# wenhao728/VORTA

Hardware: AMD Instinct MI355X
Metric: video_tokens_per_sec (routed-attention denoising step, HunyuanVideo 720p 129f) (higher is better)
Workload: dtype fp16

## Files before the change

### vorta_amd/csrc/attn_fwd.hip

```cpp
#include <hip/hip_runtime.h>
#include <stdint.h>

#include "vorta_hip.h"
#include "common.h"

#include "attn_common.h"
#include "attn_fwd_diag.inc"

namespace {
using namespace vorta_attn;

template <typename T, int NW>
__global__ __launch_bounds__(NW * 64, 2) void attn_fwd_kernel(const Params p) {
  using V8 = typename MF<T>::v8;
  using V4 = typename MF<T>::v4;
  constexpr int NT = NW * 64;
  constexpr int QB = NW * 32;
  constexpr int CH = (KVB * 16) / NT;
  constexpr int ROWSTEP = NT / 16;

  __shared__ __attribute__((aligned(16))) char smem[2 * BUF_BYTES];

  const int wg = live_order(p, blockIdx.x, gridDim.x, p.xcd_remap);
  const int sp = wg % p.n_splits;
  const int rest = wg / p.n_splits;
  const int n_qb = p.n_groups * p.blocks_per_group;
  const int qb = rest % n_qb;
  const int y = rest / n_qb;
  if (p.n_heads_dev && y >= *p.n_heads_dev) return;
  const int head = p.head_list ? p.head_list[y] : y;
  int grp, p0, pend;
  q_block_of(p, qb, QB, grp, p0, pend);

  const int tid = threadIdx.x;
  const int lane = tid & 63;
  const int wave = __builtin_amdgcn_readfirstlane(tid >> 6);
  const int r32 = lane & 31;
  const int hh = lane >> 5;

  const int n_kv = p.n_kv_dev ? max(1, min(*p.n_kv_dev, p.n_kv)) : p.n_kv;
  const int q_valid = p.q_valid_dev ? min(*p.q_valid_dev, p.q_valid) : p.q_valid;
  const int nblk_total = (n_kv + KVB - 1) / KVB;
  const int blk0 = sp * p.blocks_per_split;
  const int blk1 = min(blk0 + p.blocks_per_split, nblk_total);

  const int wrow0 = p0 + wave * 32;
  const bool wave_active = wrow0 < pend;
  const int my_p = wrow0 + r32;
  const bool row_ok = my_p < pend;
  const int ld_p = min(my_p, pend - 1);
  const int32_t* q_rows = p.q_rows ? p.q_rows + (int64_t)y * p.q_rows_sh : nullptr;
  const int64_t my_row = q_rows ? (int64_t)q_rows[ld_p] : (int64_t)(p.q_row_offset + ld_p);

  V8 qf[8];
  {
    const char* qp = p.q + (int64_t)head * p.q_sh + my_row * p.q_ss + hh * 16;
#pragma unroll
    for (int ks = 0; ks < 8; ++ks) qf[ks] = *(const V8*)(qp + ks * 32);
  }

  const int32_t* kv_rows =
      p.kv_rows ? p.kv_rows + (int64_t)y * p.kv_rows_sh + (int64_t)grp * p.kv_rows_sg : nullptr;
  const char* kbase = p.k + (int64_t)head * p.k_sh + (tid & 15) * 16;
  const char* vbase = p.v + (int64_t)head * p.v_sh + (tid & 15) * 16;
  const int lrow0 = tid >> 4;
  const int lcc = tid & 15;
  int k_wr[CH], v_wr[CH];
#pragma unroll
  for (int i = 0; i < CH; ++i) {
    const int row = lrow0 + i * ROWSTEP;
    k_wr[i] = row * ROWB + ((lcc ^ (row & 15)) << 4);
    v_wr[i] = TILE_BYTES + row * ROWB + ((lcc ^ ((row & 3) << 2)) << 4);
  }
  u32x4 kreg[CH], vreg[CH];
  int64_t nrow[CH];
#define FETCH_ROWS(blk_)                                                          \
  _Pragma("unroll") for (int i_ = 0; i_ < CH; ++i_) {                             \
    const int pos_ = min((blk_) * KVB + lrow0 + i_ * ROWSTEP, n_kv - 1);          \
    nrow[i_] = kv_rows ? (int64_t)kv_rows[pos_] : (int64_t)(p.kv_row_offset + pos_); \
  }
#define ISSUE_LOADS()                                                             \
  _Pragma("unroll") for (int i_ = 0; i_ < CH; ++i_) {                             \
    kreg[i_] = *(const u32x4*)(kbase + nrow[i_] * p.k_ss);                        \
    vreg[i_] = *(const u32x4*)(vbase + nrow[i_] * p.v_ss);                        \
  }
#define WRITE_LDS(buf_)                                                           \
  _Pragma("unroll") for (int i_ = 0; i_ < CH; ++i_) {                             \
    *(u32x4*)(smem + (buf_) * BUF_BYTES + k_wr[i_]) = kreg[i_];                   \
    *(u32x4*)(smem + (buf_) * BUF_BYTES + v_wr[i_]) = vreg[i_];                   \
  }

  int k_rd[8];
#pragma unroll
  for (int ks = 0; ks < 8; ++ks) k_rd[ks] = r32 * ROWB + (((2 * ks + hh) ^ (r32 & 15)) << 4);
  int v_rd[4];
  {
    const int g = lane >> 4, i16 = lane & 15, q4 = i16 >> 2, pp = i16 & 3;
#pragma unroll
    for (int dt = 0; dt < 4; ++dt)
      v_rd[dt] = TILE_BYTES + (4 * (g >> 1) + q4) * ROWB + ((dt ^ q4) << 6) + 32 * (g & 1) + 8 * pp;
  }

  f32x16 o[4];
#pragma unroll
  for (int dt = 0; dt < 4; ++dt)
#pragma unroll
    for (int i = 0; i < 16; ++i) o[dt][i] = 0.f;
  float m_run = -1e30f, l_run = 0.f;
  const float c = p.scale_log2;

  if (blk0 < blk1) {
    FETCH_ROWS(blk0);
    ISSUE_LOADS();
    if (blk0 + 1 < blk1) { FETCH_ROWS(blk0 + 1); }
    WRITE_LDS(0);
    if (blk0 + 1 < blk1) { ISSUE_LOADS(); }
    if (blk0 + 2 < blk1) { FETCH_ROWS(blk0 + 2); }
    __syncthreads();
  }

  for (int blk = blk0; blk < blk1; ++blk) {
    const int buf = (blk - blk0) & 1;
    const char* sb = smem + buf * BUF_BYTES;
    V8 pb[4];
    if (wave_active) {
      f32x16 s0, s1;
#pragma unroll
      for (int i = 0; i < 16; ++i) { s0[i] = 0.f; s1[i] = 0.f; }
#pragma unroll
      for (int ks = 0; ks < 8; ++ks) {
        const V8 k0 = *(const V8*)(sb + k_rd[ks]);
        const V8 k1 = *(const V8*)(sb + k_rd[ks] + 32 * ROWB);
        s0 = MF<T>::mfma(k0, qf[ks], s0);
        s1 = MF<T>::mfma(k1, qf[ks], s1);
      }
      const int kv0 = blk * KVB;
      if (kv0 + KVB > n_kv) {
#pragma unroll
        for (int i = 0; i < 16; ++i) {
          const int row = (i & 3) + 8 * (i >> 2) + 4 * hh;
          if (kv0 + row >= n_kv) s0[i] = -INFINITY;
          if (kv0 + 32 + row >= n_kv) s1[i] = -INFINITY;
        }
      }
      float mx = s0[0];
#pragma unroll
      for (int i = 1; i < 16; ++i) mx = fmaxf(mx, s0[i]);
#pragma unroll
      for (int i = 0; i < 16; ++i) mx = fmaxf(mx, s1[i]);
      mx = half_max(mx);
      const float m_new = fmaxf(m_run, mx);
      if (!__all(m_new == m_run)) {
        const float alpha = __builtin_amdgcn_exp2f((m_run - m_new) * c);
#pragma unroll
        for (int dt = 0; dt < 4; ++dt)
#pragma unroll
          for (int i = 0; i < 16; ++i) o[dt][i] *= alpha;
        l_run *= alpha;
        m_run = m_new;
      }
      const float mc = m_run * c;
      float lsum = 0.f;
#pragma unroll
      for (int i = 0; i < 16; ++i) {
        s0[i] = __builtin_amdgcn_exp2f(fmaf(s0[i], c, -mc));
        s1[i] = __builtin_amdgcn_exp2f(fmaf(s1[i], c, -mc));
        lsum += s0[i] + s1[i];
      }
      l_run += lsum;
#pragma unroll
      for (int j = 0; j < 8; ++j) {
        pb[0][j] = (T)s0[j];
        pb[1][j] = (T)s0[8 + j];
        pb[2][j] = (T)s1[j];
        pb[3][j] = (T)s1[8 + j];
      }
    }
    if (blk + 1 < blk1) {
      WRITE_LDS(buf ^ 1);
      if (blk + 2 < blk1) { ISSUE_LOADS(); }
      if (blk + 3 < blk1) { FETCH_ROWS(blk + 3); }
    }
    if (wave_active) {
#pragma unroll
      for (int dt = 0; dt < 4; ++dt) {
#pragma unroll
        for (int kg = 0; kg < 4; ++kg) {
          const V4 lo = MF<T>::tr(sb + v_rd[dt] + (16 * kg) * ROWB);
          const V4 hi = MF<T>::tr(sb + v_rd[dt] + (16 * kg + 8) * ROWB);
          V8 vf;
#pragma unroll
          for (int j = 0; j < 4; ++j) { vf[j] = lo[j]; vf[4 + j] = hi[j]; }
          o[dt] = MF<T>::mfma(vf, pb[kg], o[dt]);
        }
      }
    }
    __syncthreads();
  }

  if (!wave_active) return;
  const float l_tot = half_sum(l_run);
  if (p.n_splits > 1) {
    if (row_ok) {
      const int64_t slot = ((int64_t)y * p.n_splits + sp) * p.n_q + my_p;
      float* wo = p.ws_o + slot * D;
#pragma unroll
      for (int dt = 0; dt < 4; ++dt)
#pragma unroll
        for (int rg = 0; rg < 4; ++rg) {
          f32x4 v = {o[dt][4 * rg], o[dt][4 * rg + 1], o[dt][4 * rg + 2], o[dt][4 * rg + 3]};
          *(f32x4*)(wo + 32 * dt + 8 * rg + 4 * hh) = v;
        }
      if (hh == 0) {
        p.ws_ml[slot * 2] = m_run * c;
        p.ws_ml[slot * 2 + 1] = l_tot;
      }
    }
    return;
  }
  if (!row_ok) return;
  const float inv = (my_p < q_valid && l_tot > 0.f) ? 1.f / l_tot : 0.f;
  uint2 packed[16];
#pragma unroll
  for (int dt = 0; dt < 4; ++dt)
#pragma unroll
    for (int rg = 0; rg < 4; ++rg) {
      V4 t;
#pragma unroll
      for (int j = 0; j < 4; ++j) t[j] = (T)(o[dt][4 * rg + j] * inv);
      packed[dt * 4 + rg] = *(uint2*)&t;
    }
  char* obase = p.o + (int64_t)head * p.o_sh + hh * 8;
  auto store_row = [&](int64_t row) {
    char* op = obase + row * p.o_ss;
#pragma unroll
    for (int dt = 0; dt < 4; ++dt)
#pragma unroll
      for (int rg = 0; rg < 4; ++rg) *(uint2*)(op + (32 * dt + 8 * rg) * 2) = packed[dt * 4 + rg];
  };
  store_row(my_row);
  if (p.dup_rows && my_p < p.n_dup_pos) {
    const int32_t* dr = p.dup_rows + (int64_t)y * p.dup_rows_sh + (int64_t)my_p * p.n_dup;
    for (int i = 0; i < p.n_dup; ++i) store_row((int64_t)dr[i]);
  }
}

constexpr int RING = 2;

template <typename T, int NW, bool KVTAB, int NS>
__device__ __forceinline__ void attn_pipe_dma_body(const Params& p, char* __restrict__ smem, const int wg) {
  static_assert(NS == 2, "ring depth");
  TRACE_ENTRY_()
  using V8 = typename MF<T>::v8;
  using V4 = typename MF<T>::v4;
  constexpr int NT = NW * 64;
  constexpr int QB = NW * 32;
  constexpr int CH = (KVB * 16) / NT;
  constexpr int ROWSTEP = NT / 16;
#ifndef VORTA_KPRE
#define VORTA_KPRE 2
#endif
  constexpr int KPRE = (NW == 4 && KVTAB && VORTA_KPRE > 1) ? 1 : VORTA_KPRE;
  const int sp = wg % p.n_splits;
  const int rest = wg / p.n_splits;
  const int n_qb = p.n_groups * p.blocks_per_group;
  const int qb = rest % n_qb;
  const int y = rest / n_qb;
  if (p.n_heads_dev && y >= *p.n_heads_dev) return;
  const int head = p.head_list ? p.head_list[y] : y;
  int grp, p0, pend;
  q_block_of(p, qb, QB, grp, p0, pend);

  const int tid = threadIdx.x;
  const int lane = tid & 63;
  const int wave = __builtin_amdgcn_readfirstlane(tid >> 6);
  const int r32 = lane & 31;
  const int hh = lane >> 5;

  const int n_kv = p.n_kv_dev ? max(1, min(*p.n_kv_dev, p.n_kv)) : p.n_kv;
  const int q_valid = p.q_valid_dev ? min(*p.q_valid_dev, p.q_valid) : p.q_valid;
  const int nblk_total = (n_kv + KVB - 1) / KVB;
  const int blk0 = sp * p.blocks_per_split;
  const int blk1 = min(blk0 + p.blocks_per_split, nblk_total);

  const int wrow0 = p0 + wave * 32;
  const bool wave_active = wrow0 < pend;
  const int my_p = wrow0 + r32;
  const bool row_ok = my_p < pend;
  const int ld_p = min(my_p, pend - 1);
  const int32_t* q_rows = p.q_rows ? p.q_rows + (int64_t)y * p.q_rows_sh : nullptr;
  const int64_t my_row = q_rows ? (int64_t)q_rows[ld_p] : (int64_t)(p.q_row_offset + ld_p);

  V8 qf[8];
  {
    const char* qp = p.q + (int64_t)head * p.q_sh + my_row * p.q_ss + hh * 16;
#pragma unroll
    for (int ks = 0; ks < 8; ++ks) {
      const V8 raw = *(const V8*)(qp + ks * 32);
#pragma unroll
      for (int i = 0; i < 8; ++i) qf[ks][i] = (T)((float)raw[i] * p.scale_log2);
    }
  }

  const int32_t* kv_rows =
      p.kv_rows ? p.kv_rows + (int64_t)y * p.kv_rows_sh + (int64_t)grp * p.kv_rows_sg : nullptr;
  const char* kbase = p.k + (int64_t)head * p.k_sh + (tid & 15) * 16;
  const char* vbase = p.v + (int64_t)head * p.v_sh + (tid & 15) * 16;
  const int lrow0 = tid >> 4;
  const int lcc = tid & 15;
  const __amdgpu_buffer_rsrc_t k_rsrc = __builtin_amdgcn_make_buffer_rsrc(
      (void*)(p.k + (int64_t)head * p.k_sh), 0, 0x7fffffff, 0x00020000);
  const __amdgpu_buffer_rsrc_t v_rsrc = __builtin_amdgcn_make_buffer_rsrc(
      (void*)(p.v + (int64_t)head * p.v_sh), 0, 0x7fffffff, 0x00020000);
  const int k_ss32 = (int)p.k_ss, v_ss32 = (int)p.v_ss;
  int k_col[CH], v_col[CH];
#pragma unroll
  for (int i = 0; i < CH; ++i) {
    const int row = 4 * (CH * wave + i) + (lane >> 4);
    k_col[i] = ((lane & 15) ^ (row & 15)) << 4;
    v_col[i] = ((lane & 15) ^ ((row & 3) << 2)) << 4;
  }
  int rowK[CH], rowV[CH];
  int posK[CH];
#define ROWS_OF(dst_, blk_)                                                       \
  _Pragma("unroll") for (int i_ = 0; i_ < CH; ++i_) {                             \
    const int pos_ = min((blk_) * KVB + 4 * (CH * wave + i_) + (lane >> 4), n_kv - 1); \
    if constexpr (KVTAB) dst_[i_] = kv_rows[pos_];                                \
    else dst_[i_] = p.kv_row_offset + pos_;                                       \
  }
#define DMA_K(par_) _Pragma("unroll") for (int i_ = 0; i_ < CH; ++i_) __builtin_amdgcn_raw_ptr_buffer_load_lds(   \
      k_rsrc, (LDS_AS void*)(smem + (par_) * TILE_BYTES + (CH * wave + i_) * 1024), 16,                            \
      (int)__umul24((unsigned)rowK[i_], (unsigned)k_ss32) + k_col[i_], 0, 0, 0);
#define DMA_V(par_) _Pragma("unroll") for (int i_ = 0; i_ < CH; ++i_) __builtin_amdgcn_raw_ptr_buffer_load_lds(   \
      v_rsrc, (LDS_AS void*)(smem + (NS + (par_)) * TILE_BYTES + (CH * wave + i_) * 1024), 16,                     \
      (int)__umul24((unsigned)rowV[i_], (unsigned)v_ss32) + v_col[i_], 0, 0, 0);

  int k_rd[8];
#pragma unroll
  for (int ks = 0; ks < 8; ++ks) k_rd[ks] = r32 * ROWB + (((2 * ks + hh) ^ (r32 & 15)) << 4);
  int v_rd[4];
  {
    const int g = lane >> 4, i16 = lane & 15, q4 = i16 >> 2, pp = i16 & 3;
#pragma unroll
    for (int dt = 0; dt < 4; ++dt)
      v_rd[dt] = NS * TILE_BYTES + (4 * (g >> 1) + q4) * ROWB + ((dt ^ q4) << 6) + 32 * (g & 1) + 8 * pp;
  }

  f32x16 o[4];
#pragma unroll
  for (int dt = 0; dt < 4; ++dt)
#pragma unroll
    for (int i = 0; i < 16; ++i) o[dt][i] = 0.f;
  float m_run = -1e30f, l_run = 0.f;
  const float defer = p.defer_log2;
  f32x16 sA0, sA1, sB0, sB1;
  f32x16 minit;
#pragma unroll
  for (int i = 0; i < 16; ++i) minit[i] = 0.f;
  float mx_cur = -1e30f;

#define QK(d0_, d1_, par_)                                                        \
  {                                                                               \
    _Pragma("unroll") for (int ks_ = 0; ks_ < 8; ++ks_) {                         \
      const V8 k0_ = *(const V8*)(smem + (par_) * TILE_BYTES + k_rd[ks_]);        \
      const V8 k1_ = *(const V8*)(smem + (par_) * TILE_BYTES + k_rd[ks_] + 32 * ROWB); \
      d0_ = MF<T>::mfma(k0_, qf[ks_], ks_ == 0 ? minit : d0_);                    \
      d1_ = MF<T>::mfma(k1_, qf[ks_], ks_ == 0 ? minit : d1_);                    \
    }                                                                             \
  }
#define ROW_MAX(dst_, a_, b_)                                                      \
  {                                                                               \
    float mx_ = a_[0];                                                            \
    _Pragma("unroll") for (int i_ = 1; i_ < 16; ++i_) mx_ = fmaxf(mx_, a_[i_]);   \
    _Pragma("unroll") for (int i_ = 0; i_ < 16; ++i_) mx_ = fmaxf(mx_, b_[i_]);   \
    dst_ = half_max(mx_);                                                         \
  }
#define ROW_MAX_POS(dst_, a_, b_)                                                  \
  {                                                                               \
    int m0_ = max(max(__float_as_int(a_[0]), __float_as_int(a_[1])), __float_as_int(a_[2])); \
    int m1_ = max(max(__float_as_int(b_[0]), __float_as_int(b_[1])), __float_as_int(b_[2])); \
    _Pragma("unroll") for (int i_ = 3; i_ < 15; i_ += 2) {                        \
      m0_ = max(max(m0_, __float_as_int(a_[i_])), __float_as_int(a_[i_ + 1]));    \
      m1_ = max(max(m1_, __float_as_int(b_[i_])), __float_as_int(b_[i_ + 1]));    \
    }                                                                             \
    m0_ = max(max(m0_, __float_as_int(a_[15])), __float_as_int(b_[15]));          \
    m0_ = max(m0_, m1_);                                                          \
    auto r_ = __builtin_amdgcn_permlane32_swap((unsigned)m0_, (unsigned)m0_, false, false); \
    dst_ = __int_as_float(max((int)r_[0], (int)r_[1]));                           \
  }
#define QK_PRE(d0_, d1_, par_)                                                    \
  {                                                                               \
    _Pragma("unroll") for (int ks_ = 0; ks_ < 8; ++ks_) {                         \
      V8 k0_, k1_;                                                                \
      if (ks_ < KPRE) { k0_ = kpre_[ks_][0]; k1_ = kpre_[ks_][1]; }               \
      else {                                                                      \
        k0_ = *(const V8*)(smem + (par_) * TILE_BYTES + k_rd[ks_]);               \
        k1_ = *(const V8*)(smem + (par_) * TILE_BYTES + k_rd[ks_] + 32 * ROWB);   \
      }                                                                           \
      d0_ = MF<T>::mfma(k0_, qf[ks_], ks_ == 0 ? minit : d0_);                    \
      d1_ = MF<T>::mfma(k1_, qf[ks_], ks_ == 0 ? minit : d1_);                    \
    }                                                                             \
  }
#define RAISE_REF(g_, c0_, c1_)                                                   \
  {                                                                               \
    const float alpha_ = __builtin_amdgcn_exp2f(-(g_));                           \
    _Pragma("unroll") for (int dt_ = 0; dt_ < 4; ++dt_)                           \
      _Pragma("unroll") for (int i_ = 0; i_ < 16; ++i_) o[dt_][i_] *= alpha_;     \
    l_run *= alpha_;                                                              \
    m_run += (g_);                                                                \
    _Pragma("unroll") for (int i_ = 0; i_ < 16; ++i_) { c0_[i_] -= (g_); c1_[i_] -= (g_); minit[i_] = -m_run; } \
    asm volatile("" : "+v"(minit));                                               \
  }
#define STAGE_DMA(kfree_, vfree_, j_)                                             \
  DMA_K(kfree_)                                                                   \
  DMA_V(vfree_)                                                                   \
  _Pragma("unroll") for (int i_ = 0; i_ < CH; ++i_) rowV[i_] = rowK[i_];          \
  if constexpr (NW == 8) {                                                        \
    _Pragma("unroll") for (int i_ = 0; i_ < CH; ++i_) {                           \
      posK[i_] += KVB;                                                            \
      const int pos_ = min(posK[i_], n_kv - 1);                                   \
      if constexpr (KVTAB) rowK[i_] = kv_rows[pos_];                              \
      else rowK[i_] = p.kv_row_offset + pos_;                                     \
    }                                                                             \
  } else {  \
    ROWS_OF(rowK, (j_) + NS + 1)                                                  \
  }                                                                               \
  __builtin_amdgcn_sched_barrier(0);
  TRACE_VARS_()
#ifndef STEP_SYNC
#define STEP_SYNC() asm volatile("s_waitcnt vmcnt(0) lgkmcnt(0)\n\ts_barrier" ::: "memory");
#endif

#ifndef VORTA_SCHED
#define VORTA_SCHED 1
#endif
#if VORTA_SCHED == 1
#define SCHED_RECIPE()                                                            \
  _Pragma("unroll") for (int g_ = 0; g_ < 16; ++g_) {                             \
    __builtin_amdgcn_sched_group_barrier(0x008, 1, 0);                            \
    __builtin_amdgcn_sched_group_barrier(0x100, 1, 0);                            \
    __builtin_amdgcn_sched_group_barrier(0x400, 2, 0);                            \
    __builtin_amdgcn_sched_group_barrier(0x002, 2, 0);                            \
  }                                                                               \
  _Pragma("unroll") for (int g_ = 0; g_ < 16; ++g_) {                             \
    __builtin_amdgcn_sched_group_barrier(0x008, 1, 0);                            \
    __builtin_amdgcn_sched_group_barrier(0x100, 2, 0);                            \
    __builtin_amdgcn_sched_group_barrier(0x002, 4, 0);                            \
  }
#else
#define SCHED_RECIPE()
#endif
#define STEP(c0_, c1_, n0_, n1_, kcur_, knext_, vfree_, j_)                       \
  {  \
    STAGE_DMA(kcur_, vfree_, j_)                                                  \
    STEP_BODY(c0_, c1_, n0_, n1_, kcur_, knext_, j_)                              \
    STEP_SYNC()                                                                   \
  }
#define STEP_BODY(c0_, c1_, n0_, n1_, kcur_, knext_, j_)                          \
  {                                                                               \
    if (wave_active) {                                                            \
      V8 kpre_[KPRE > 0 ? KPRE : 1][2];                                                          \
      _Pragma("unroll") for (int ks_ = 0; ks_ < KPRE; ++ks_) {                    \
        kpre_[ks_][0] = *(const V8*)(smem + (knext_) * TILE_BYTES + k_rd[ks_]);   \
        kpre_[ks_][1] = *(const V8*)(smem + (knext_) * TILE_BYTES + k_rd[ks_] + 32 * ROWB); \
      }                                                                           \
       \
       \
      if ((j_) * KVB + KVB > n_kv) {                                              \
        int h4_ = 4 * hh;  \
        asm volatile("" : "+v"(h4_));                                             \
        _Pragma("unroll") for (int i_ = 0; i_ < 16; ++i_) {                       \
          const int row_ = (i_ & 3) + 8 * (i_ >> 2) + h4_;                        \
          if ((j_) * KVB + row_ >= n_kv) c0_[i_] = -INFINITY;                     \
          if ((j_) * KVB + 32 + row_ >= n_kv) c1_[i_] = -INFINITY;                \
        }                                                                         \
        ROW_MAX(mx_cur, c0_, c1_)                                                 \
      }                                                                           \
       \
       \
       \
      if (!__all(mx_cur <= defer)) {                                              \
        const float g_ = fmaxf(mx_cur, 0.f);                                      \
        RAISE_REF(g_, c0_, c1_)                                                   \
      }                                                                           \
      V8 pb_[4];                                                                  \
      QK_PRE(n0_, n1_, knext_)     \
      float lsum_ = 0.f;                                                          \
      _Pragma("unroll") for (int i_ = 0; i_ < 16; ++i_) {                         \
        c0_[i_] = __builtin_amdgcn_exp2f(c0_[i_]);                                \
        c1_[i_] = __builtin_amdgcn_exp2f(c1_[i_]);                                \
        lsum_ += c0_[i_] + c1_[i_];                                               \
      }                                                                           \
      l_run += lsum_;                                                             \
      _Pragma("unroll") for (int e_ = 0; e_ < 8; ++e_) {                          \
        pb_[0][e_] = (T)c0_[e_];                                                  \
        pb_[1][e_] = (T)c0_[8 + e_];                                              \
        pb_[2][e_] = (T)c1_[e_];                                                  \
        pb_[3][e_] = (T)c1_[8 + e_];                                              \
      }                                                                           \
      _Pragma("unroll") for (int dt_ = 0; dt_ < 4; ++dt_) {                       \
        _Pragma("unroll") for (int kg_ = 0; kg_ < 4; ++kg_) {                     \
          const V4 lo_ = MF<T>::tr(smem + (kcur_) * TILE_BYTES + v_rd[dt_] + (16 * kg_) * ROWB); \
          const V4 hi_ = MF<T>::tr(smem + (kcur_) * TILE_BYTES + v_rd[dt_] + (16 * kg_ + 8) * ROWB); \
          V8 vf_;                                                                 \
          _Pragma("unroll") for (int e_ = 0; e_ < 4; ++e_) { vf_[e_] = lo_[e_]; vf_[4 + e_] = hi_[e_]; } \
          o[dt_] = MF<T>::mfma(vf_, pb_[kg_], o[dt_]);                            \
        }                                                                         \
      }                                                                           \
      ROW_MAX_POS(mx_cur, n0_, n1_)  \
      SCHED_RECIPE()                                                              \
    }                                                                             \
  }

  if (blk0 < blk1) {
    ROWS_OF(rowK, blk0)
    _Pragma("unroll") for (int i_ = 0; i_ < CH; ++i_) rowV[i_] = rowK[i_];
    DMA_K(0)
    DMA_V(0)
    ROWS_OF(rowK, blk0 + 1)
    DMA_K(1)
    _Pragma("unroll") for (int i_ = 0; i_ < CH; ++i_) rowV[i_] = rowK[i_];
    ROWS_OF(rowK, blk0 + NS)
    _Pragma("unroll") for (int i_ = 0; i_ < CH; ++i_) posK[i_] = (blk0 + NS) * KVB + 4 * (CH * wave + i_) + (lane >> 4);
    __syncthreads();
    if (wave_active) {
      QK(sA0, sA1, 0)
      if (blk0 * KVB + KVB > n_kv) {
#pragma unroll
        for (int i = 0; i < 16; ++i) {
          const int row = (i & 3) + 8 * (i >> 2) + 4 * hh;
          if (blk0 * KVB + row >= n_kv) sA0[i] = -INFINITY;
          if (blk0 * KVB + 32 + row >= n_kv) sA1[i] = -INFINITY;
        }
      }
      ROW_MAX(mx_cur, sA0, sA1)
      m_run = mx_cur;
#pragma unroll
      for (int i = 0; i < 16; ++i) { sA0[i] -= m_run; sA1[i] -= m_run; minit[i] = -m_run; }
      asm volatile("" : "+v"(minit));
      mx_cur = 0.f;
    }
    __syncthreads();
  }
  for (int blk = blk0; blk < blk1; blk += 2) {
    STEP(sA0, sA1, sB0, sB1, 0, 1, 1, blk)
    if (blk + 1 >= blk1) break;
    STEP(sB0, sB1, sA0, sA1, 1, 0, 0, blk + 1)
  }
#undef QK
#undef QK_PRE
#undef ROW_MAX
#undef ROW_MAX_POS
#undef RAISE_REF
#undef STEP
#undef STEP_BODY
#undef STAGE_DMA
#undef STEP_SYNC
#undef ROWS_OF
#undef DMA_K
#undef DMA_V

  TRACE_FLUSH_()
  if (!wave_active) return;
  const float l_tot = half_sum(l_run);
  if (p.n_splits > 1) {
    if (row_ok) {
      const int64_t slot = ((int64_t)y * p.n_splits + sp) * p.n_q + my_p;
      float* wo = p.ws_o + slot * D;
#pragma unroll
      for (int dt = 0; dt < 4; ++dt)
#pragma unroll
        for (int rg = 0; rg < 4; ++rg) {
          f32x4 v = {o[dt][4 * rg], o[dt][4 * rg + 1], o[dt][4 * rg + 2], o[dt][4 * rg + 3]};
          *(f32x4*)(wo + 32 * dt + 8 * rg + 4 * hh) = v;
        }
      if (hh == 0) {
        p.ws_ml[slot * 2] = m_run;
        p.ws_ml[slot * 2 + 1] = l_tot;
      }
    }
    return;
  }
  if (!row_ok) return;
  const float inv = (my_p < q_valid && l_tot > 0.f) ? 1.f / l_tot : 0.f;
  uint2 packed[16];
#pragma unroll
  for (int dt = 0; dt < 4; ++dt)
#pragma unroll
    for (int rg = 0; rg < 4; ++rg) {
      V4 t;
#pragma unroll
      for (int j = 0; j < 4; ++j) t[j] = (T)(o[dt][4 * rg + j] * inv);
      packed[dt * 4 + rg] = *(uint2*)&t;
    }
  char* obase = p.o + (int64_t)head * p.o_sh + hh * 8;
  auto store_row = [&](int64_t row) {
    char* op = obase + row * p.o_ss;
#pragma unroll
    for (int dt = 0; dt < 4; ++dt)
#pragma unroll
      for (int rg = 0; rg < 4; ++rg) *(uint2*)(op + (32 * dt + 8 * rg) * 2) = packed[dt * 4 + rg];
  };
  store_row(my_row);
  if (p.dup_rows && my_p < p.n_dup_pos) {
    const int32_t* dr = p.dup_rows + (int64_t)y * p.dup_rows_sh + (int64_t)my_p * p.n_dup;
    for (int i = 0; i < p.n_dup; ++i) store_row((int64_t)dr[i]);
  }
}


template <typename T, int NW, bool KVTAB>
__global__ __launch_bounds__(NW * 64, 2) void attn_fwd_pipe_kernel(const Params p) {
#if defined(__HIP_DEVICE_COMPILE__)
  constexpr int NS = RING;
  __shared__ __attribute__((aligned(16))) char smem[2 * NS * TILE_BYTES];
  const int wg = live_order(p, blockIdx.x, gridDim.x, p.xcd_remap);
  attn_pipe_dma_body<T, NW, KVTAB, NS>(p, smem, wg);
#endif
}


template <typename T>
__global__ __launch_bounds__(512, 2) void attn_fwd_multi_kernel(const MultiOf<Params> mp) {
#if defined(__HIP_DEVICE_COMPILE__)
  __shared__ __attribute__((aligned(16))) char smem[2 * RING * TILE_BYTES];
  int wg;
  const Params& p = segment_of(mp, blockIdx.x, wg);
  if (p.kv_rows) attn_pipe_dma_body<T, 8, true, RING>(p, smem, wg);
  else attn_pipe_dma_body<T, 8, false, RING>(p, smem, wg);
#endif
}

}

int vorta_attn::fill_params(const vorta_attn_args* a, Params& p, int& block_rows, int in_esize, int v_esize, int k_esize) {
  if (v_esize == 0) v_esize = in_esize;
  if (k_esize == 0) k_esize = in_esize;
  if (!a || a->struct_size != sizeof(vorta_attn_args)) return VORTA_EINVAL;
  if (in_esize == 2 ? (a->dtype != VORTA_BF16 && a->dtype != VORTA_FP16) : a->dtype != VORTA_FP8E4M3) return VORTA_EUNSUPPORTED;
  if (a->head_dim != D) return VORTA_EUNSUPPORTED;
  if (a->n_heads < 0 || a->n_q < 0 || a->n_kv < 0) return VORTA_EINVAL;
  if (a->n_heads == 0 || a->n_q == 0) { block_rows = 0; p.n_groups = 0; p.blocks_per_group = 0; p.n_heads = 0; return VORTA_OK; }
  if (a->n_kv == 0) return VORTA_EINVAL;
  if (!a->q.ptr || !a->k.ptr || !a->v.ptr || !a->o.ptr) return VORTA_EINVAL;
  const vorta_tensor* ts[4] = {&a->q, &a->k, &a->v, &a->o};
  for (int i = 0; i < 4; ++i) {
    const vorta_tensor* t = ts[i];
    const int al = 16 / (i == 0 ? in_esize : i == 1 ? k_esize : i == 2 ? v_esize : 2);
    if (((uintptr_t)t->ptr & 15) || (t->stride_s % al) || (t->stride_h % al) || t->stride_s < D) return VORTA_EINVAL;
  }
  if (a->n_splits < 1 || a->n_splits > 1024) return VORTA_EINVAL;
  if (!(a->scale > 0.f)) return VORTA_EINVAL;
  if (a->n_splits > 1 && (!a->ws_o || !a->ws_ml)) return VORTA_EINVAL;
  if (a->q_group_len < 0 || a->q_valid < 0) return VORTA_EINVAL;
  if (a->dup_rows && (a->n_dup < 0 || a->n_dup_pos < 0 || a->n_dup_pos > a->n_q)) return VORTA_EINVAL;
  if (a->block_rows != 0 && a->block_rows != 128 && a->block_rows != 256) return VORTA_EINVAL;
  if (a->variant < 0 || a->variant > 2) return VORTA_EINVAL;
  if (a->variant != 1 && (a->k.stride_s * k_esize >= (1 << 24) || a->v.stride_s * v_esize >= (1 << 24))) return VORTA_EUNSUPPORTED;
  if (a->variant != 1 && !a->kv_rows) {
    const int64_t last = (int64_t)a->kv_row_offset + a->n_kv;
    const int64_t ks = a->k.stride_s * k_esize, vs = a->v.stride_s * v_esize;
    const int64_t ss = ks > vs ? ks : vs;
    if (last >= (1 << 24) || last * ss > 0x7fffffffll) return VORTA_EUNSUPPORTED;
  }
  p.q = (const char*)a->q.ptr; p.k = (const char*)a->k.ptr; p.v = (const char*)a->v.ptr; p.o = (char*)a->o.ptr;
  p.q_sh = a->q.stride_h * in_esize; p.k_sh = a->k.stride_h * k_esize; p.v_sh = a->v.stride_h * v_esize; p.o_sh = a->o.stride_h * 2;
  p.q_ss = a->q.stride_s * in_esize; p.k_ss = a->k.stride_s * k_esize; p.v_ss = a->v.stride_s * v_esize; p.o_ss = a->o.stride_s * 2;
  p.head_list = a->head_list; p.n_heads_dev = a->n_heads_dev; p.n_heads = a->n_heads;
  p.n_q = a->n_q; p.q_group_len = a->q_group_len > 0 ? a->q_group_len : a->n_q;
  p.q_row_offset = a->q_row_offset; p.q_valid = a->q_valid;
  p.q_rows = a->q_rows; p.q_rows_sh = a->q_rows_stride_h;
  p.n_kv = a->n_kv; p.kv_row_offset = a->kv_row_offset;
  p.n_kv_dev = a->n_kv_dev; p.q_valid_dev = a->q_valid_dev;
  p.kv_rows = a->kv_rows; p.kv_rows_sh = a->kv_rows_stride_h; p.kv_rows_sg = a->kv_rows_stride_g;
  p.dup_rows = a->dup_rows; p.dup_rows_sh = a->dup_rows_stride_h; p.n_dup_pos = a->n_dup_pos; p.n_dup = a->n_dup;
  p.scale_log2 = a->scale * 1.4426950408889634f;
  p.n_splits = a->n_splits; p.ws_o = a->ws_o; p.ws_ml = a->ws_ml;
  p.xcd_remap = (a->reserved & 1) ? 0 : 1;
  p.defer_log2 = (a->reserved & 4) ? 0.f : 6.f;
  p.n_groups = (p.n_q + p.q_group_len - 1) / p.q_group_len;
  block_rows = a->block_rows;
  if (block_rows == 0) {
    const int g = p.q_group_len;
    const int64_t pad256 = ((g + 255) / 256) * 256, pad128 = ((g + 127) / 128) * 128;
    block_rows = (pad256 * 100 > pad128 * 106) ? 128 : 256;
  }
  p.blocks_per_group = (p.q_group_len + block_rows - 1) / block_rows;
  p.q_block_table = a->q_block_table;
  if (a->q_block_table) {
    if (a->n_q_blocks <= 0 || (a->block_rows != 128 && a->block_rows != 256)) return VORTA_EINVAL;
    p.n_groups = a->n_q_blocks;
    p.blocks_per_group = 1;
  }
  const int nblk = (p.n_kv + KVB - 1) / KVB;
  p.blocks_per_split = (nblk + p.n_splits - 1) / p.n_splits;
  p.wg_per_slot = p.n_groups * p.blocks_per_group * p.n_splits;
  return VORTA_OK;
}

namespace {
using namespace vorta_attn;

struct Family16 {
  using PP = Params;
  int fill(const vorta_attn_args* a, Params& p, int& block_rows) const { return fill_params(a, p, block_rows, 2); }
  bool fusable(const vorta_attn_args& a, const Params&) const { return a.variant != 1; }
  int out_dtype(const vorta_attn_args& a) const { return a.dtype; }
  template <typename T> static constexpr auto multi = attn_fwd_multi_kernel<T>;
  template <typename T> static auto kernel(const vorta_attn_args& a, const Params& p, int block_rows) {
    if (a.variant == 1) return block_rows == 256 ? attn_fwd_kernel<T, 8> : attn_fwd_kernel<T, 4>;
    if (block_rows == 256) return p.kv_rows ? attn_fwd_pipe_kernel<T, 8, true> : attn_fwd_pipe_kernel<T, 8, false>;
    return p.kv_rows ? attn_fwd_pipe_kernel<T, 4, true> : attn_fwd_pipe_kernel<T, 4, false>;
  }
};
}

extern "C" int vorta_attn_workspace_bytes(const vorta_attn_args* a, uint64_t* ws_o_bytes, uint64_t* ws_ml_bytes) {
  if (!a || a->struct_size != sizeof(vorta_attn_args) || !ws_o_bytes || !ws_ml_bytes) return VORTA_EINVAL;
  if (a->n_splits <= 1) { *ws_o_bytes = 0; *ws_ml_bytes = 0; return VORTA_OK; }
  const uint64_t slots = (uint64_t)a->n_heads * (uint64_t)a->n_splits * (uint64_t)a->n_q;
  *ws_o_bytes = slots * D * sizeof(float);
  *ws_ml_bytes = slots * 2 * sizeof(float);
  return VORTA_OK;
}

extern "C" int vorta_attn_plan(const vorta_attn_args* a, int32_t* block_rows_out, int64_t* n_workgroups_out,
                               int32_t* kernel_id_out) {
  Params p{};
  int block_rows = 0;
  int rc = vorta_attn::fill_params(a, p, block_rows, (a && a->dtype == VORTA_FP8E4M3) ? 1 : 2);
  if (rc != VORTA_OK) return rc;
  if (block_rows_out) *block_rows_out = block_rows;
  if (kernel_id_out) {
    const bool pipe = a->variant != 1;
    *kernel_id_out = (block_rows == 256 ? 8 : 4) * 16 + (pipe ? 1 : 0) + ((pipe && a->kv_rows) ? 2 : 0);
  }
  if (n_workgroups_out) *n_workgroups_out = (int64_t)p.n_groups * p.blocks_per_group * p.n_heads * (p.n_heads ? p.n_splits : 0);
  return VORTA_OK;
}

extern "C" int vorta_attn_fwd_batch(const vorta_attn_args* args, int32_t n, void* hip_stream) {
  return fwd_batch(Family16{}, args, n, hip_stream);
}

extern "C" int vorta_attn_fwd(const vorta_attn_args* a, void* hip_stream) { return fwd_single(Family16{}, a, hip_stream); }
```

Baseline: 29230.

## Split attention KV loop into unclamped steady-state and clamped tail phases

The main KV loop now runs a steady-state phase over whole blocks, followed by a tail phase. The steady state skips the position clamp and the boundary masking. For the contiguous (non-table) case it also advances precomputed buffer offsets by a fixed stride instead of recomputing row*stride products each step. The epilogue recomputes lane, row and half indices from threadIdx so those values need not stay live in registers through the loop. The aim is to cut per-iteration scalar/vector ALU work and register pressure, at the cost of more code paths and a trickier boundary handoff between the phases.

After: 29570 (median of 6 runs). 1.2% higher.

```diff
diff --git a/vorta_amd/csrc/attn_fwd.hip b/vorta_amd/csrc/attn_fwd.hip
--- a/vorta_amd/csrc/attn_fwd.hip
+++ b/vorta_amd/csrc/attn_fwd.hip
@@ -286,7 +286,6 @@
   const int wrow0 = p0 + wave * 32;
   const bool wave_active = wrow0 < pend;
   const int my_p = wrow0 + r32;
-  const bool row_ok = my_p < pend;
   const int ld_p = min(my_p, pend - 1);
   const int32_t* q_rows = p.q_rows ? p.q_rows + (int64_t)y * p.q_rows_sh : nullptr;
   const int64_t my_row = q_rows ? (int64_t)q_rows[ld_p] : (int64_t)(p.q_row_offset + ld_p);
@@ -322,18 +321,23 @@
   }
   int rowK[CH], rowV[CH];
   int posK[CH];
-#define ROWS_OF(dst_, blk_)                                                       \
+  unsigned offK[CH], offV[CH];
+  const unsigned k_step = (unsigned)(KVB * k_ss32), v_step = (unsigned)(KVB * v_ss32);
+#define ROWS_OF(dst_, blk_, clamp_)                                               \
   _Pragma("unroll") for (int i_ = 0; i_ < CH; ++i_) {                             \
-    const int pos_ = min((blk_) * KVB + 4 * (CH * wave + i_) + (lane >> 4), n_kv - 1); \
+    int pos_ = (blk_) * KVB + 4 * (CH * wave + i_) + (lane >> 4);                 \
+    if constexpr (clamp_) pos_ = min(pos_, n_kv - 1);                             \
     if constexpr (KVTAB) dst_[i_] = kv_rows[pos_];                                \
     else dst_[i_] = p.kv_row_offset + pos_;                                       \
   }
-#define DMA_K(par_) _Pragma("unroll") for (int i_ = 0; i_ < CH; ++i_) __builtin_amdgcn_raw_ptr_buffer_load_lds(   \
-      k_rsrc, (LDS_AS void*)(smem + (par_) * TILE_BYTES + (CH * wave + i_) * 1024), 16,                            \
-      (int)__umul24((unsigned)rowK[i_], (unsigned)k_ss32) + k_col[i_], 0, 0, 0);
-#define DMA_V(par_) _Pragma("unroll") for (int i_ = 0; i_ < CH; ++i_) __builtin_amdgcn_raw_ptr_buffer_load_lds(   \
-      v_rsrc, (LDS_AS void*)(smem + (NS + (par_)) * TILE_BYTES + (CH * wave + i_) * 1024), 16,                     \
-      (int)__umul24((unsigned)rowV[i_], (unsigned)v_ss32) + v_col[i_], 0, 0, 0);
+#define K_OFF(i_) ((int)__umul24((unsigned)rowK[i_], (unsigned)k_ss32) + k_col[i_])
+#define V_OFF(i_) ((int)__umul24((unsigned)rowV[i_], (unsigned)v_ss32) + v_col[i_])
+#define DMA_K_AT(par_, off_) _Pragma("unroll") for (int i_ = 0; i_ < CH; ++i_) __builtin_amdgcn_raw_ptr_buffer_load_lds( \
+      k_rsrc, (LDS_AS void*)(smem + (par_) * TILE_BYTES + (CH * wave + i_) * 1024), 16, (int)(off_), 0, 0, 0);
+#define DMA_V_AT(par_, off_) _Pragma("unroll") for (int i_ = 0; i_ < CH; ++i_) __builtin_amdgcn_raw_ptr_buffer_load_lds( \
+      v_rsrc, (LDS_AS void*)(smem + (NS + (par_)) * TILE_BYTES + (CH * wave + i_) * 1024), 16, (int)(off_), 0, 0, 0);
+#define DMA_K(par_) DMA_K_AT(par_, K_OFF(i_))
+#define DMA_V(par_) DMA_V_AT(par_, V_OFF(i_))
 
   int k_rd[8];
 #pragma unroll
@@ -411,19 +415,25 @@
     _Pragma("unroll") for (int i_ = 0; i_ < 16; ++i_) { c0_[i_] -= (g_); c1_[i_] -= (g_); minit[i_] = -m_run; } \
     asm volatile("" : "+v"(minit));                                               \
   }
-#define STAGE_DMA(kfree_, vfree_, j_)                                             \
-  DMA_K(kfree_)                                                                   \
-  DMA_V(vfree_)                                                                   \
-  _Pragma("unroll") for (int i_ = 0; i_ < CH; ++i_) rowV[i_] = rowK[i_];          \
-  if constexpr (NW == 8) {                                                        \
-    _Pragma("unroll") for (int i_ = 0; i_ < CH; ++i_) {                           \
-      posK[i_] += KVB;                                                            \
-      const int pos_ = min(posK[i_], n_kv - 1);                                   \
-      if constexpr (KVTAB) rowK[i_] = kv_rows[pos_];                              \
-      else rowK[i_] = p.kv_row_offset + pos_;                                     \
+#define STAGE_DMA(kfree_, vfree_, j_, tail_)                                      \
+  if constexpr (!KVTAB && !(tail_)) {                                             \
+    DMA_K_AT(kfree_, offK[i_])                                                    \
+    DMA_V_AT(vfree_, offV[i_])                                                    \
+    _Pragma("unroll") for (int i_ = 0; i_ < CH; ++i_) { offK[i_] += k_step; offV[i_] += v_step; } \
+  } else {                                                                        \
+    DMA_K(kfree_)                                                                 \
+    DMA_V(vfree_)                                                                 \
+    _Pragma("unroll") for (int i_ = 0; i_ < CH; ++i_) rowV[i_] = rowK[i_];        \
+    if constexpr (NW == 8) {                                                      \
+      _Pragma("unroll") for (int i_ = 0; i_ < CH; ++i_) {                         \
+        posK[i_] += KVB;                                                          \
+        const int pos_ = (tail_) ? min(posK[i_], n_kv - 1) : posK[i_];            \
+        if constexpr (KVTAB) rowK[i_] = kv_rows[pos_];                            \
+        else rowK[i_] = p.kv_row_offset + pos_;                                   \
+      }                                                                           \
+    } else {  \
+      ROWS_OF(rowK, (j_) + NS + 1, tail_)                                         \
     }                                                                             \
-  } else {  \
-    ROWS_OF(rowK, (j_) + NS + 1)                                                  \
   }                                                                               \
   __builtin_amdgcn_sched_barrier(0);
   TRACE_VARS_()
@@ -450,13 +460,13 @@
 #else
 #define SCHED_RECIPE()
 #endif
-#define STEP(c0_, c1_, n0_, n1_, kcur_, knext_, vfree_, j_)                       \
+#define STEP(c0_, c1_, n0_, n1_, kcur_, knext_, vfree_, j_, tail_)                \
   {  \
-    STAGE_DMA(kcur_, vfree_, j_)                                                  \
-    STEP_BODY(c0_, c1_, n0_, n1_, kcur_, knext_, j_)                              \
+    STAGE_DMA(kcur_, vfree_, j_, tail_)                                           \
+    STEP_BODY(c0_, c1_, n0_, n1_, kcur_, knext_, j_, tail_)                       \
     STEP_SYNC()                                                                   \
   }
-#define STEP_BODY(c0_, c1_, n0_, n1_, kcur_, knext_, j_)                          \
+#define STEP_BODY(c0_, c1_, n0_, n1_, kcur_, knext_, j_, tail_)                   \
   {                                                                               \
     if (wave_active) {                                                            \
       V8 kpre_[KPRE > 0 ? KPRE : 1][2];                                                          \
@@ -466,7 +476,7 @@
       }                                                                           \
        \
        \
-      if ((j_) * KVB + KVB > n_kv) {                                              \
+      if ((tail_) && (j_) * KVB + KVB > n_kv) {                                   \
         int h4_ = 4 * hh;  \
         asm volatile("" : "+v"(h4_));                                             \
         _Pragma("unroll") for (int i_ = 0; i_ < 16; ++i_) {                       \
@@ -513,15 +523,18 @@
   }
 
   if (blk0 < blk1) {
-    ROWS_OF(rowK, blk0)
+    ROWS_OF(rowK, blk0, true)
     _Pragma("unroll") for (int i_ = 0; i_ < CH; ++i_) rowV[i_] = rowK[i_];
     DMA_K(0)
     DMA_V(0)
-    ROWS_OF(rowK, blk0 + 1)
+    ROWS_OF(rowK, blk0 + 1, true)
     DMA_K(1)
     _Pragma("unroll") for (int i_ = 0; i_ < CH; ++i_) rowV[i_] = rowK[i_];
-    ROWS_OF(rowK, blk0 + NS)
+    ROWS_OF(rowK, blk0 + NS, true)
     _Pragma("unroll") for (int i_ = 0; i_ < CH; ++i_) posK[i_] = (blk0 + NS) * KVB + 4 * (CH * wave + i_) + (lane >> 4);
+    if constexpr (!KVTAB) {
+      _Pragma("unroll") for (int i_ = 0; i_ < CH; ++i_) { offK[i_] = (unsigned)K_OFF(i_); offV[i_] = (unsigned)V_OFF(i_); }
+    }
     __syncthreads();
     if (wave_active) {
       QK(sA0, sA1, 0)
@@ -542,10 +555,23 @@
     }
     __syncthreads();
   }
-  for (int blk = blk0; blk < blk1; blk += 2) {
-    STEP(sA0, sA1, sB0, sB1, 0, 1, 1, blk)
+  const int blk_whole = min(blk1, n_kv / KVB - (KVTAB ? NS + 1 : NS));
+  int blk = blk0;
+  for (; blk + 1 < blk_whole; blk += 2) {
+    STEP(sA0, sA1, sB0, sB1, 0, 1, 1, blk, false)
+    STEP(sB0, sB1, sA0, sA1, 1, 0, 0, blk + 1, false)
+  }
+  if constexpr (!KVTAB) {
+    if (blk > blk0 && blk < blk1) {
+      ROWS_OF(rowV, blk + 1, true)
+      ROWS_OF(rowK, blk + NS, true)
+      _Pragma("unroll") for (int i_ = 0; i_ < CH; ++i_) posK[i_] = (blk + NS) * KVB + 4 * (CH * wave + i_) + (lane >> 4);
+    }
+  }
+  for (; blk < blk1; blk += 2) {
+    STEP(sA0, sA1, sB0, sB1, 0, 1, 1, blk, true)
     if (blk + 1 >= blk1) break;
-    STEP(sB0, sB1, sA0, sA1, 1, 0, 0, blk + 1)
+    STEP(sB0, sB1, sA0, sA1, 1, 0, 0, blk + 1, true)
   }
 #undef QK
 #undef QK_PRE
@@ -559,30 +585,40 @@
 #undef ROWS_OF
 #undef DMA_K
 #undef DMA_V
+#undef DMA_K_AT
+#undef DMA_V_AT
+#undef K_OFF
+#undef V_OFF
 
   TRACE_FLUSH_()
   if (!wave_active) return;
+  int tid_e = threadIdx.x;
+  asm volatile("" : "+v"(tid_e));
+  const int hh_e = (tid_e >> 5) & 1;
+  const int e_p = wrow0 + (tid_e & 31);
+  const bool e_ok = e_p < pend;
+  const int64_t e_row = q_rows ? (int64_t)q_rows[min(e_p, pend - 1)] : (int64_t)(p.q_row_offset + min(e_p, pend - 1));
   const float l_tot = half_sum(l_run);
   if (p.n_splits > 1) {
-    if (row_ok) {
-      const int64_t slot = ((int64_t)y * p.n_splits + sp) * p.n_q + my_p;
+    if (e_ok) {
+      const int64_t slot = ((int64_t)y * p.n_splits + sp) * p.n_q + e_p;
       float* wo = p.ws_o + slot * D;
 #pragma unroll
       for (int dt = 0; dt < 4; ++dt)
 #pragma unroll
         for (int rg = 0; rg < 4; ++rg) {
           f32x4 v = {o[dt][4 * rg], o[dt][4 * rg + 1], o[dt][4 * rg + 2], o[dt][4 * rg + 3]};
-          *(f32x4*)(wo + 32 * dt + 8 * rg + 4 * hh) = v;
+          *(f32x4*)(wo + 32 * dt + 8 * rg + 4 * hh_e) = v;
         }
-      if (hh == 0) {
+      if (hh_e == 0) {
         p.ws_ml[slot * 2] = m_run;
         p.ws_ml[slot * 2 + 1] = l_tot;
       }
     }
     return;
   }
-  if (!row_ok) return;
-  const float inv = (my_p < q_valid && l_tot > 0.f) ? 1.f / l_tot : 0.f;
+  if (!e_ok) return;
+  const float inv = (e_p < q_valid && l_tot > 0.f) ? 1.f / l_tot : 0.f;
   uint2 packed[16];
 #pragma unroll
   for (int dt = 0; dt < 4; ++dt)
@@ -593,7 +629,7 @@
       for (int j = 0; j < 4; ++j) t[j] = (T)(o[dt][4 * rg + j] * inv);
       packed[dt * 4 + rg] = *(uint2*)&t;
     }
-  char* obase = p.o + (int64_t)head * p.o_sh + hh * 8;
+  char* obase = p.o + (int64_t)head * p.o_sh + hh_e * 8;
   auto store_row = [&](int64_t row) {
     char* op = obase + row * p.o_ss;
 #pragma unroll
@@ -601,9 +637,9 @@
 #pragma unroll
       for (int rg = 0; rg < 4; ++rg) *(uint2*)(op + (32 * dt + 8 * rg) * 2) = packed[dt * 4 + rg];
   };
-  store_row(my_row);
-  if (p.dup_rows && my_p < p.n_dup_pos) {
-    const int32_t* dr = p.dup_rows + (int64_t)y * p.dup_rows_sh + (int64_t)my_p * p.n_dup;
+  store_row(e_row);
+  if (p.dup_rows && e_p < p.n_dup_pos) {
+    const int32_t* dr = p.dup_rows + (int64_t)y * p.dup_rows_sh + (int64_t)e_p * p.n_dup;
     for (int i = 0; i < p.n_dup; ++i) store_row((int64_t)dr[i]);
   }
 }
```
